# LikeLy-Journey/SegmenTron

Hardware: AMD Instinct MI355X
Metric: images/sec fwd+bwd DeepLabv3+_xception65 @1025x2049 (higher is better)
Workload: dtype bf16; 1 GPU; DeepLabv3+_xception65 train step (fwd + CE loss + bwd + SGD) @1025x2049, batch 2/GPU (BASELINE.json configs[2]); global_batch=2, bn=BN, parallelism=dp1, full_size=True

## Files before the change

segmentron_amd/csrc/dwconv_row.hip:

```cpp
#include "common.h"
#include "dwconv.h"

namespace seg {

constexpr int RW_THREADS = 256, RW_CQ = 8, RW_PL = RW_THREADS / RW_CQ, RW_CH = RW_CQ * 4;

struct DwRowArgs {
  const void* src;
  const void* xc;
  void* out;
  const float* w;
  const float* sc; const float* sh;
  float* partial_a;
  float* partial_bn;
  long ldsrc, ldxc, ldout;
  int N, H, W, C, dil, pro_mode, TW, ntw, ntiles;
};

template <typename T, bool BWD>
__global__ __launch_bounds__(RW_THREADS, BWD ? 2 : 3) void dwconv_row_kernel(const DwRowArgs a) {
  using V = Vec<T>;
  using H4 = HVec<T>;
  constexpr int VN = V::N, VPP = RW_CH / VN;
  constexpr int NACC = BWD ? 9 : 2;
  extern __shared__ __attribute__((aligned(16))) unsigned char rw_smem[];
  T* tile = reinterpret_cast<T*>(rw_smem);
  const int tid = threadIdx.x;
  const int flat = blockIdx.x + gridDim.x * blockIdx.y;
  const int L = xcd_remap(flat, gridDim.x * gridDim.y);
  const int by = L / (int)gridDim.x, bx = L - by * (int)gridDim.x;
  const int cq = tid & (RW_CQ - 1), pl = tid / RW_CQ;
  const int cbase = bx * RW_CH;
  const int c0 = cbase + cq * 4;
  const bool cok = c0 < a.C;
  const int c0s = cok ? c0 : 0;
  const int d = a.dil, TWH = a.TW + 2 * d;
  const T* __restrict__ SRC = reinterpret_cast<const T*>(a.src);
  const T* __restrict__ XC = reinterpret_cast<const T*>(a.xc);
  T* __restrict__ OUT = reinterpret_cast<T*>(a.out);

  const int sv = tid % VPP;
  const int sc0 = cbase + sv * VN;
  const bool sok = sc0 < a.C;
  float ps[VN], pt[VN];
#pragma unroll
  for (int i = 0; i < VN; ++i) { ps[i] = 1.f; pt[i] = 0.f; }
  float sc[4], sh[4];
#pragma unroll
  for (int i = 0; i < 4; ++i) { sc[i] = 1.f; sh[i] = 0.f; }
  if (a.pro_mode & PRO_AFFINE) {
    if (!BWD) {
      load_params<VN>(a.sc, sok ? sc0 : 0, ps);
      load_params<VN>(a.sh, sok ? sc0 : 0, pt);
    } else {
      load_params<4>(a.sc, c0s, sc);
      load_params<4>(a.sh, c0s, sh);
    }
  }
  float wv[9][4];
#pragma unroll
  for (int k = 0; k < 9; ++k) load_params<4>(a.w + (long)k * a.C, c0s, wv[k]);
  float acc[NACC][4], s1[4], s2[4];
#pragma unroll
  for (int k = 0; k < NACC; ++k)
#pragma unroll
    for (int i = 0; i < 4; ++i) acc[k][i] = 0.f;
#pragma unroll
  for (int i = 0; i < 4; ++i) s1[i] = s2[i] = 0.f;

  const int nph = d < a.H ? d : a.H;
  const int nvec_row = TWH * VPP;
  for (int t = by; t < a.ntiles; t += gridDim.y) {
    const int tw = t % a.ntw, tq = t / a.ntw;
    const int ph = tq % nph, n = tq / nph;
    const int w0 = tw * a.TW;
    auto stage_row = [&](int slot, int hh) {
      T* dst = tile + (long)slot * TWH * RW_CH;
      const bool rok = sok && hh >= 0 && hh < a.H;
      for (int idx = tid; idx < nvec_row; idx += RW_THREADS) {
        const int px = idx / VPP;
        const int ww = w0 - d + px;
        const bool ok = rok && ww >= 0 && ww < a.W;
        uint4 v = ldg16(SRC + (ok ? (((long)n * a.H + hh) * a.W + ww) * a.ldsrc + sc0 : 0));
        if (!BWD && a.pro_mode != PRO_NONE) {
          float f[VN];
          V::unpack(v, f);
          apply_prologue_regs<VN>(f, a.pro_mode, ps, pt);
          v = V::pack(f);
        }
        v = mask_u4(v, ok);
        *reinterpret_cast<uint4*>(dst + (long)px * RW_CH + sv * VN) = v;
      }
    };
    __syncthreads();
    stage_row(0, ph - d);
    stage_row(1, ph);
    int k = 0;
    for (int h = ph; h < a.H; h += d, ++k) {
      const long orow = ((long)n * a.H + h) * a.W;
      constexpr int MAXP = (160 + RW_PL - 1) / RW_PL;
      typename H4::raw_t xraw[MAXP];
      if (BWD) {
#pragma unroll
        for (int q = 0; q < MAXP; ++q) {
          const int p = pl + q * RW_PL;
          const bool ok = cok && p < a.TW && w0 + p < a.W;
          xraw[q] = H4::load_raw(XC + (ok ? (orow + w0 + p) * a.ldxc + c0 : 0));
        }
      }
      stage_row((k + 2) % 3, h + d);
      __syncthreads();
      const T* slot_of[3] = {tile + (long)(k % 3) * TWH * RW_CH,
                             tile + (long)((k + 1) % 3) * TWH * RW_CH,
                             tile + (long)((k + 2) % 3) * TWH * RW_CH};
#pragma unroll
      for (int q = 0; q < MAXP; ++q) {
        const int p = pl + q * RW_PL;
        if (!(cok && p < a.TW && w0 + p < a.W)) continue;
        const long poff = (long)(p + d) * RW_CH + cq * 4;
        float o[4] = {0.f, 0.f, 0.f, 0.f};
        if (!BWD) {
#pragma unroll
          for (int kh = 0; kh < 3; ++kh)
#pragma unroll
            for (int kw = 0; kw < 3; ++kw) {
              float f[4];
              H4::load(slot_of[kh] + poff + (long)(kw - 1) * d * RW_CH, f);
#pragma unroll
              for (int i = 0; i < 4; ++i) o[i] = fmaf(f[i], wv[kh * 3 + kw][i], o[i]);
            }
          H4::store(OUT + (orow + w0 + p) * a.ldout + c0, o);
#pragma unroll
          for (int i = 0; i < 4; ++i) {
            acc[0][i] += o[i];
            acc[1][i] = fmaf(o[i], o[i], acc[1][i]);
          }
        } else {
          float xr[4], xa[4];
          H4::unpack_raw(xraw[q], xr);
#pragma unroll
          for (int i = 0; i < 4; ++i) {
            float v = xr[i];
            if (a.pro_mode & PRO_AFFINE) v = fmaf(v, sc[i], sh[i]);
            if (a.pro_mode & PRO_RELU) v = fmaxf(v, 0.f);
            if (a.pro_mode & PRO_CLAMP6) v = fminf(v, 6.f);
            xa[i] = v;
          }
#pragma unroll
          for (int kh = 0; kh < 3; ++kh)
#pragma unroll
            for (int kw = 0; kw < 3; ++kw) {
              float f[4];
              H4::load(slot_of[2 - kh] + poff - (long)(kw - 1) * d * RW_CH, f);
#pragma unroll
              for (int i = 0; i < 4; ++i) {
                o[i] = fmaf(f[i], wv[kh * 3 + kw][i], o[i]);
                acc[kh * 3 + kw][i] = fmaf(f[i], xa[i], acc[kh * 3 + kw][i]);
              }
            }
          if (a.pro_mode & PRO_RELU) {
#pragma unroll
            for (int i = 0; i < 4; ++i) {
              const bool on = xa[i] > 0.f && (!(a.pro_mode & PRO_CLAMP6) || xa[i] < 6.f);
              o[i] = on ? o[i] : 0.f;
            }
          }
          H4::store(OUT + (orow + w0 + p) * a.ldout + c0, o);
#pragma unroll
          for (int i = 0; i < 4; ++i) {
            s1[i] += o[i];
            s2[i] = fmaf(o[i], xr[i], s2[i]);
          }
        }
      }
      __syncthreads();
    }
  }

  constexpr int NR = BWD ? 11 : 2;
  float r[NR][4];
#pragma unroll
  for (int k = 0; k < NACC; ++k)
#pragma unroll
    for (int i = 0; i < 4; ++i) r[k][i] = acc[k][i];
  if (BWD) {
#pragma unroll
    for (int i = 0; i < 4; ++i) { r[NR - 2][i] = s1[i]; r[NR - 1][i] = s2[i]; }
  }
#pragma unroll
  for (int k = 0; k < NR; ++k)
#pragma unroll
    for (int i = 0; i < 4; ++i) {
#pragma unroll
      for (int m = RW_CQ; m < 64; m <<= 1) r[k][i] += __shfl_xor(r[k][i], m, 64);
    }
  __syncthreads();
  float* red = reinterpret_cast<float*>(rw_smem);
  const int wave = tid >> 6;
  if ((tid & 63) < RW_CQ) {
#pragma unroll
    for (int k = 0; k < NR; ++k)
#pragma unroll
      for (int i = 0; i < 4; ++i) red[((wave * RW_CQ + cq) * NR + k) * 4 + i] = r[k][i];
  }
  __syncthreads();
  for (int e = tid; e < RW_CQ * NR * 4; e += RW_THREADS) {
    float tot = 0.f;
#pragma unroll
    for (int wv4 = 0; wv4 < 4; ++wv4) tot += red[wv4 * RW_CQ * NR * 4 + e];
    const int lq = e / (NR * 4), k = (e / 4) % NR, i = e & 3;
    const int c = cbase + lq * 4 + i;
    if (c >= a.C) continue;
    if (!BWD) {
      if (a.partial_a != nullptr) a.partial_a[((long)by * 2 + k) * a.C + c] = tot;
    } else if (k < 9) {
      a.partial_a[((long)by * 9 + k) * a.C + c] = tot;
    } else if (a.partial_bn != nullptr) {
      a.partial_bn[((long)by * 2 + (k - 9)) * a.C + c] = tot;
    }
  }
}

constexpr size_t RW_LDS_MAX = 120 * 1024;

static void row_geom(int dtype, int W, int dil, int& TW, int& ntw) {
  const size_t px_bytes = (size_t)3 * RW_CH * (dtype == DT_BF16 ? 2 : 4);
  ntw = (W + 159) / 160;
  for (;;) {
    TW = (W + ntw - 1) / ntw;
    if ((size_t)(TW + 2 * dil) * px_bytes <= RW_LDS_MAX || TW == 1) break;
    ++ntw;
  }
}

int dw_row_grid_y(int dtype, int C, int N, int H, int W, int dil) {
  int TW, ntw;
  row_geom(dtype, W, dil, TW, ntw);
  const long ntiles = (long)N * (dil < H ? dil : H) * ntw;
  const int gx = (C + RW_CH - 1) / RW_CH;
  long cap = 768 / gx;
  if (cap < 1) cap = 1;
  return (int)(ntiles < cap ? ntiles : cap);
}

template <typename T, bool BWD>
static int launch_row(DwRowArgs a, int dtype, int grid_y, hipStream_t st) {
  row_geom(dtype, a.W, a.dil, a.TW, a.ntw);
  a.ntiles = a.N * (a.dil < a.H ? a.dil : a.H) * a.ntw;
  const size_t tile_b = (size_t)3 * (a.TW + 2 * a.dil) * RW_CH * sizeof(T);
  const size_t red_b = (size_t)4 * RW_CQ * (BWD ? 11 : 2) * 4 * sizeof(float);
  const size_t lds = tile_b > red_b ? tile_b : red_b;
  SEG_REQUIRE(lds <= RW_LDS_MAX, "dwconv3x3 (row): %zu bytes of LDS for dil=%d", lds, a.dil);
  static const int once = (int)hipFuncSetAttribute(
      reinterpret_cast<const void*>(&dwconv_row_kernel<T, BWD>),
      hipFuncAttributeMaxDynamicSharedMemorySize, (int)RW_LDS_MAX);
  if (once != 0) {
    set_error("dwconv3x3 (row): cannot reserve %zu bytes of LDS", RW_LDS_MAX);
    return 2;
  }
  const dim3 grid((a.C + RW_CH - 1) / RW_CH, grid_y);
  hipLaunchKernelGGL((dwconv_row_kernel<T, BWD>), grid, dim3(RW_THREADS), lds, st, a);
  return check_launch(BWD ? "dwconv3x3_bwd_fused (row)" : "dwconv3x3 (row)");
}

int launch_dw_row_fwd(int dtype, const void* x, long ldx, int N, int H, int W, int C,
                      const float* w9c, int dil, int pro_mode, const float* sc, const float* sh,
                      void* y, long ldy, float* stat_partial, int grid_y, hipStream_t st) {
  SEG_REQUIRE(grid_y == dw_row_grid_y(dtype, C, N, H, W, dil), "dwconv3x3 (row): grid_y %d != %d",
              grid_y, dw_row_grid_y(dtype, C, N, H, W, dil));
  DwRowArgs a = {};
  a.src = x; a.out = y; a.w = w9c; a.sc = sc; a.sh = sh; a.partial_a = stat_partial;
  a.ldsrc = ldx; a.ldout = ldy; a.N = N; a.H = H; a.W = W; a.C = C; a.dil = dil;
  a.pro_mode = pro_mode;
  if (dtype == DT_BF16) return launch_row<bf16_t, false>(a, dtype, grid_y, st);
  return launch_row<float, false>(a, dtype, grid_y, st);
}

int launch_dw_row_bwd(int dtype, const void* dy, long lddy, const void* x, long ldx, int N, int H,
                      int W, int C, const float* w9c, int dil, int pro_mode, const float* sc,
                      const float* sh, void* g, long ldg, float* partial_w, float* partial_bn,
                      int grid_y, hipStream_t st) {
  SEG_REQUIRE(grid_y == dw_row_grid_y(dtype, C, N, H, W, dil),
              "dwconv3x3_bwd_fused (row): grid_y %d != %d", grid_y,
              dw_row_grid_y(dtype, C, N, H, W, dil));
  DwRowArgs a = {};
  a.src = dy; a.xc = x; a.out = g; a.w = w9c; a.sc = sc; a.sh = sh;
  a.partial_a = partial_w; a.partial_bn = partial_bn;
  a.ldsrc = lddy; a.ldxc = ldx; a.ldout = ldg; a.N = N; a.H = H; a.W = W; a.C = C; a.dil = dil;
  a.pro_mode = pro_mode;
  if (dtype == DT_BF16) return launch_row<bf16_t, true>(a, dtype, grid_y, st);
  return launch_row<float, true>(a, dtype, grid_y, st);
}

}
```

Baseline: 92.21 images/sec.

## Software-pipeline row dwconv with register-staged loads, 4-slot LDS ring, LDS taps

Reworks the row-tiled depthwise 3x3 kernel so the global loads for the next input row go into registers before the current row's compute, and are written to LDS only afterward. A 4-slot LDS ring is used when it fits, which removes one barrier per row. For bf16 backward, the 9 taps and the BN affine are moved from registers into LDS so three blocks can fit per CU instead of two. Output stores are deferred until after compute and offsets become 32-bit. The cost is more template variants (NV), more code complexity, and extra LDS reads per tap in the backward path.

```diff
diff --git a/segmentron_amd/csrc/dwconv_row.hip b/segmentron_amd/csrc/dwconv_row.hip
--- a/segmentron_amd/csrc/dwconv_row.hip
+++ b/segmentron_amd/csrc/dwconv_row.hip
@@ -1,9 +1,13 @@
+#include <type_traits>
+
 #include "common.h"
 #include "dwconv.h"
 
 namespace seg {
 
 constexpr int RW_THREADS = 256, RW_CQ = 8, RW_PL = RW_THREADS / RW_CQ, RW_CH = RW_CQ * 4;
+constexpr int RW_MAXTW = 160, RW_MAXDIL = 64;
+constexpr int RW_MAXTWH = RW_MAXTW + 2 * RW_MAXDIL;
 
 struct DwRowArgs {
   const void* src;
@@ -14,17 +18,43 @@
   float* partial_a;
   float* partial_bn;
   long ldsrc, ldxc, ldout;
-  int N, H, W, C, dil, pro_mode, TW, ntw, ntiles;
+  int N, H, W, C, dil, pro_mode, TW, ntw, ntiles, nslot;
 };
 
-template <typename T, bool BWD>
-__global__ __launch_bounds__(RW_THREADS, BWD ? 2 : 3) void dwconv_row_kernel(const DwRowArgs a) {
+#ifndef RW_BWD_BF16_BLOCKS
+#define RW_BWD_BF16_BLOCKS 3
+#endif
+#ifndef RW_RING_SLOTS
+#define RW_RING_SLOTS 4
+#endif
+template <typename T, bool BWD, int NV> constexpr int row_blocks_per_cu() {
+  if (sizeof(T) == 4) return (BWD || NV > 6) ? 2 : 3;
+  return BWD ? RW_BWD_BF16_BLOCKS : 3;
+}
+template <typename T, bool BWD> constexpr bool row_taps_in_lds() {
+  return BWD && sizeof(T) == 2 && RW_BWD_BF16_BLOCKS == 3;
+}
+
+__device__ __forceinline__ int opaque(int v) {
+  asm volatile("" : "+v"(v));
+  return v;
+}
+
+__device__ __forceinline__ void arrived(const uint4& v) {
+  asm volatile("" ::"v"(v.x), "v"(v.y), "v"(v.z), "v"(v.w));
+}
+__device__ __forceinline__ void arrived(const uint2& v) { asm volatile("" ::"v"(v.x), "v"(v.y)); }
+
+template <typename T, bool BWD, int NV>
+__global__ __launch_bounds__(RW_THREADS, (row_blocks_per_cu<T, BWD, NV>())) void dwconv_row_kernel(const DwRowArgs a) {
+  constexpr bool WLDS = row_taps_in_lds<T, BWD>();
   using V = Vec<T>;
   using H4 = HVec<T>;
+  using raw_t = typename H4::raw_t;
   constexpr int VN = V::N, VPP = RW_CH / VN;
   constexpr int NACC = BWD ? 9 : 2;
+  constexpr int MAXP = (RW_MAXTW + RW_PL - 1) / RW_PL;
   extern __shared__ __attribute__((aligned(16))) unsigned char rw_smem[];
-  T* tile = reinterpret_cast<T*>(rw_smem);
   const int tid = threadIdx.x;
   const int flat = blockIdx.x + gridDim.x * blockIdx.y;
   const int L = xcd_remap(flat, gridDim.x * gridDim.y);
@@ -34,7 +64,10 @@
   const int c0 = cbase + cq * 4;
   const bool cok = c0 < a.C;
   const int c0s = cok ? c0 : 0;
-  const int d = a.dil, TWH = a.TW + 2 * d;
+  const int d = a.dil, TWH = a.TW + 2 * d, ns = a.nslot;
+  const int slot_elems = TWH * RW_CH;
+  T* tile = reinterpret_cast<T*>(rw_smem);
+  float* wl = reinterpret_cast<float*>(rw_smem + (size_t)ns * slot_elems * sizeof(T));
   const T* __restrict__ SRC = reinterpret_cast<const T*>(a.src);
   const T* __restrict__ XC = reinterpret_cast<const T*>(a.xc);
   T* __restrict__ OUT = reinterpret_cast<T*>(a.out);
@@ -52,14 +85,23 @@
     if (!BWD) {
       load_params<VN>(a.sc, sok ? sc0 : 0, ps);
       load_params<VN>(a.sh, sok ? sc0 : 0, pt);
-    } else {
+    } else if (!WLDS) {
       load_params<4>(a.sc, c0s, sc);
       load_params<4>(a.sh, c0s, sh);
     }
   }
-  float wv[9][4];
-#pragma unroll
-  for (int k = 0; k < 9; ++k) load_params<4>(a.w + (long)k * a.C, c0s, wv[k]);
+  float wv[WLDS ? 1 : 9][4];
+  if constexpr (!WLDS) {
+#pragma unroll
+    for (int k = 0; k < 9; ++k) load_params<4>(a.w + (long)k * a.C, c0s, wv[k]);
+  } else if (tid < 11 * RW_CQ) {
+    const int k = tid / RW_CQ, q = tid % RW_CQ;
+    const int c = cbase + q * 4;
+    float t4[4] = {0.f, 0.f, 0.f, 0.f};
+    if (k < 9) load_params<4>(a.w + (long)k * a.C, c < a.C ? c : 0, t4);
+    else if (a.pro_mode & PRO_AFFINE) load_params<4>(k == 9 ? a.sc : a.sh, c < a.C ? c : 0, t4);
+    *reinterpret_cast<float4*>(wl + k * RW_CH + q * 4) = make_float4(t4[0], t4[1], t4[2], t4[3]);
+  }
   float acc[NACC][4], s1[4], s2[4];
 #pragma unroll
   for (int k = 0; k < NACC; ++k)
@@ -74,62 +116,104 @@
     const int tw = t % a.ntw, tq = t / a.ntw;
     const int ph = tq % nph, n = tq / nph;
     const int w0 = tw * a.TW;
-    auto stage_row = [&](int slot, int hh) {
-      T* dst = tile + (long)slot * TWH * RW_CH;
-      const bool rok = sok && hh >= 0 && hh < a.H;
-      for (int idx = tid; idx < nvec_row; idx += RW_THREADS) {
-        const int px = idx / VPP;
-        const int ww = w0 - d + px;
-        const bool ok = rok && ww >= 0 && ww < a.W;
-        uint4 v = ldg16(SRC + (ok ? (((long)n * a.H + hh) * a.W + ww) * a.ldsrc + sc0 : 0));
-        if (!BWD && a.pro_mode != PRO_NONE) {
-          float f[VN];
-          V::unpack(v, f);
-          apply_prologue_regs<VN>(f, a.pro_mode, ps, pt);
-          v = V::pack(f);
+    auto stage_load = [&](uint4 (&v)[NV], int hh) {
+      const char* rowp = reinterpret_cast<const char*>(SRC + ((long)n * a.H + hh) * a.W * a.ldsrc);
+      const int tv = opaque(tid);
+      const int svc = cbase + (tv % VPP) * VN;
+#pragma unroll
+      for (int j = 0; j < NV; ++j) {
+        const int idx = tv + j * RW_THREADS;
+        const int ww = w0 - d + idx / VPP;
+        const bool ok = svc < a.C && idx < nvec_row && ww >= 0 && ww < a.W;
+        const unsigned off = ok ? (unsigned)(ww * (int)a.ldsrc + svc) * (unsigned)sizeof(T) : 0u;
+        v[j] = ldg16(rowp + off);
+      }
+    };
+    auto stage_write = [&](const uint4 (&v)[NV], bool row_in, int slot) {
+      if (row_in) {
+#pragma unroll
+        for (int j = 0; j < NV; ++j) arrived(v[j]);
+      }
+      const int tv = opaque(tid);
+      T* dst = tile + slot * slot_elems + tv * VN;
+#pragma unroll
+      for (int j = 0; j < NV; ++j) {
+        const int idx = tv + j * RW_THREADS;
+        if (idx < nvec_row) {
+          uint4 o = make_uint4(0u, 0u, 0u, 0u);
+          if (row_in) {
+            const int ww = w0 - d + idx / VPP;
+            o = v[j];
+            if (!BWD && a.pro_mode != PRO_NONE) {
+              float f[VN];
+              V::unpack(o, f);
+              apply_prologue_regs<VN>(f, a.pro_mode, ps, pt);
+              o = V::pack(f);
+            }
+            o = mask_u4(o, cbase + (tv % VPP) * VN < a.C && ww >= 0 && ww < a.W);
+          }
+          *reinterpret_cast<uint4*>(dst + j * (RW_THREADS / VPP) * RW_CH) = o;
         }
-        v = mask_u4(v, ok);
-        *reinterpret_cast<uint4*>(dst + (long)px * RW_CH + sv * VN) = v;
       }
     };
+    auto load_x = [&](raw_t (&xr)[MAXP], int h) {
+      const char* rowp = reinterpret_cast<const char*>(XC + (((long)n * a.H + h) * a.W + w0) * a.ldxc);
+      const int tv = opaque(tid);
+      const int cx = cbase + (tv & (RW_CQ - 1)) * 4;
+#pragma unroll
+      for (int q = 0; q < MAXP; ++q) {
+        const int p = tv / RW_CQ + q * RW_PL;
+        const bool ok = cx < a.C && p < a.TW && w0 + p < a.W;
+        const unsigned off = ok ? (unsigned)(p * (int)a.ldxc + cx) * (unsigned)sizeof(T) : 0u;
+        xr[q] = H4::load_raw(reinterpret_cast<const T*>(rowp + off));
+      }
+    };
+
+    uint4 rv[NV];
+    raw_t xcur[BWD ? MAXP : 1];
+    {
+      uint4 rv2[NV];
+      const bool in2 = ph + d < a.H;
+      stage_load(rv, ph);
+      if (in2) stage_load(rv2, ph + d);
+      if constexpr (BWD) load_x(xcur, ph);
+      stage_write(rv, false, 0);
+      stage_write(rv, true, 1);
+      stage_write(rv2, in2, 2);
+    }
     __syncthreads();
-    stage_row(0, ph - d);
-    stage_row(1, ph);
-    int k = 0;
-    for (int h = ph; h < a.H; h += d, ++k) {
+    int r = 0;
+    auto step = [&](auto in3_c, int h) {
+      constexpr bool IN3 = decltype(in3_c)::value;
+      const int r1 = r + 1 < ns ? r + 1 : r + 1 - ns, r2 = r + 2 < ns ? r + 2 : r + 2 - ns;
+      const int r3 = r + 3 < ns ? r + 3 : r + 3 - ns;
+      const bool more = IN3 || h + d < a.H;
       const long orow = ((long)n * a.H + h) * a.W;
-      constexpr int MAXP = (160 + RW_PL - 1) / RW_PL;
-      typename H4::raw_t xraw[MAXP];
-      if (BWD) {
-#pragma unroll
-        for (int q = 0; q < MAXP; ++q) {
-          const int p = pl + q * RW_PL;
-          const bool ok = cok && p < a.TW && w0 + p < a.W;
-          xraw[q] = H4::load_raw(XC + (ok ? (orow + w0 + p) * a.ldxc + c0 : 0));
-        }
-      }
-      stage_row((k + 2) % 3, h + d);
-      __syncthreads();
-      const T* slot_of[3] = {tile + (long)(k % 3) * TWH * RW_CH,
-                             tile + (long)((k + 1) % 3) * TWH * RW_CH,
-                             tile + (long)((k + 2) % 3) * TWH * RW_CH};
+      if constexpr (IN3) stage_load(rv, h + 2 * d);
+      const T* slot_of[3] = {tile + r * slot_elems, tile + r1 * slot_elems, tile + r2 * slot_elems};
+      raw_t og[MAXP];
+      if constexpr (BWD) {
+#pragma unroll
+        for (int q = 0; q < MAXP; ++q) arrived(xcur[q]);
+      }
 #pragma unroll
       for (int q = 0; q < MAXP; ++q) {
-        const int p = pl + q * RW_PL;
+        const int tv = opaque(tid);
+        const int p = tv / RW_CQ + q * RW_PL;
         if (!(cok && p < a.TW && w0 + p < a.W)) continue;
-        const long poff = (long)(p + d) * RW_CH + cq * 4;
+        const int poff = (p + d) * RW_CH + (tv & (RW_CQ - 1)) * 4;
         float o[4] = {0.f, 0.f, 0.f, 0.f};
-        if (!BWD) {
+        asm volatile("" ::: "memory");
+        if constexpr (!BWD) {
 #pragma unroll
           for (int kh = 0; kh < 3; ++kh)
 #pragma unroll
             for (int kw = 0; kw < 3; ++kw) {
               float f[4];
-              H4::load(slot_of[kh] + poff + (long)(kw - 1) * d * RW_CH, f);
+              H4::load(slot_of[kh] + poff + (kw - 1) * d * RW_CH, f);
 #pragma unroll
               for (int i = 0; i < 4; ++i) o[i] = fmaf(f[i], wv[kh * 3 + kw][i], o[i]);
             }
-          H4::store(OUT + (orow + w0 + p) * a.ldout + c0, o);
 #pragma unroll
           for (int i = 0; i < 4; ++i) {
             acc[0][i] += o[i];
@@ -137,7 +221,15 @@
           }
         } else {
           float xr[4], xa[4];
-          H4::unpack_raw(xraw[q], xr);
+          H4::unpack_raw(xcur[q], xr);
+          if constexpr (WLDS) {
+            if (a.pro_mode & PRO_AFFINE) {
+              const float4 s4 = *reinterpret_cast<const float4*>(wl + 9 * RW_CH + (tv & (RW_CQ - 1)) * 4);
+              const float4 h4 = *reinterpret_cast<const float4*>(wl + 10 * RW_CH + (tv & (RW_CQ - 1)) * 4);
+              sc[0] = s4.x; sc[1] = s4.y; sc[2] = s4.z; sc[3] = s4.w;
+              sh[0] = h4.x; sh[1] = h4.y; sh[2] = h4.z; sh[3] = h4.w;
+            }
+          }
 #pragma unroll
           for (int i = 0; i < 4; ++i) {
             float v = xr[i];
@@ -147,17 +239,27 @@
             xa[i] = v;
           }
 #pragma unroll
-          for (int kh = 0; kh < 3; ++kh)
+          for (int kh = 0; kh < 3; ++kh) {
 #pragma unroll
             for (int kw = 0; kw < 3; ++kw) {
               float f[4];
-              H4::load(slot_of[2 - kh] + poff - (long)(kw - 1) * d * RW_CH, f);
+              H4::load(slot_of[2 - kh] + poff - (kw - 1) * d * RW_CH, f);
+              float wk[4];
+              if constexpr (WLDS) {
+                const float4 w4 = *reinterpret_cast<const float4*>(wl + (kh * 3 + kw) * RW_CH + (tv & (RW_CQ - 1)) * 4);
+                wk[0] = w4.x; wk[1] = w4.y; wk[2] = w4.z; wk[3] = w4.w;
+              } else {
+#pragma unroll
+                for (int i = 0; i < 4; ++i) wk[i] = wv[WLDS ? 0 : kh * 3 + kw][i];
+              }
 #pragma unroll
               for (int i = 0; i < 4; ++i) {
-                o[i] = fmaf(f[i], wv[kh * 3 + kw][i], o[i]);
+                o[i] = fmaf(f[i], wk[i], o[i]);
                 acc[kh * 3 + kw][i] = fmaf(f[i], xa[i], acc[kh * 3 + kw][i]);
               }
             }
+            if constexpr (WLDS) __builtin_amdgcn_sched_barrier(0);
+          }
           if (a.pro_mode & PRO_RELU) {
 #pragma unroll
             for (int i = 0; i < 4; ++i) {
@@ -165,16 +267,35 @@
               o[i] = on ? o[i] : 0.f;
             }
           }
-          H4::store(OUT + (orow + w0 + p) * a.ldout + c0, o);
 #pragma unroll
           for (int i = 0; i < 4; ++i) {
             s1[i] += o[i];
             s2[i] = fmaf(o[i], xr[i], s2[i]);
           }
         }
+        og[q] = H4::pack_raw(o);
+      }
+      if (more) {
+        if (ns == 3) __syncthreads();
+        stage_write(rv, IN3, r3);
+      }
+      char* outp = reinterpret_cast<char*>(OUT + (orow + w0) * a.ldout);
+      const int tvd = opaque(tid);
+#pragma unroll
+      for (int q = 0; q < MAXP; ++q) {
+        const int p = tvd / RW_CQ + q * RW_PL;
+        if (!(cok && p < a.TW && w0 + p < a.W)) continue;
+        *reinterpret_cast<raw_t*>(outp + (unsigned)(p * (int)a.ldout + c0) * (unsigned)sizeof(T)) = og[q];
+      }
+      if constexpr (BWD) {
+        if (more) load_x(xcur, h + d);
       }
       __syncthreads();
-    }
+      r = r1;
+    };
+    int h = ph;
+    for (; h + 2 * d < a.H; h += d) step(std::true_type{}, h);
+    for (; h < a.H; h += d) step(std::false_type{}, h);
   }
 
   constexpr int NR = BWD ? 11 : 2;
@@ -222,6 +343,8 @@
 }
 
 constexpr size_t RW_LDS_MAX = 120 * 1024;
+constexpr size_t RW_LDS_THIRD = 52 * 1024;
+constexpr size_t RW_TAPS_B = (size_t)11 * RW_CH * sizeof(float);
 
 static void row_geom(int dtype, int W, int dil, int& TW, int& ntw) {
   const size_t px_bytes = (size_t)3 * RW_CH * (dtype == DT_BF16 ? 2 : 4);
@@ -243,24 +366,42 @@
   return (int)(ntiles < cap ? ntiles : cap);
 }
 
+template <typename T, bool BWD, int NV>
+static int launch_row_nv(const DwRowArgs& a, size_t lds, const dim3& grid, hipStream_t st) {
+  static const int once = (int)hipFuncSetAttribute(
+      reinterpret_cast<const void*>(&dwconv_row_kernel<T, BWD, NV>),
+      hipFuncAttributeMaxDynamicSharedMemorySize, (int)(RW_LDS_MAX + RW_TAPS_B));
+  if (once != 0) {
+    set_error("dwconv3x3 (row): cannot reserve %zu bytes of LDS", RW_LDS_MAX + RW_TAPS_B);
+    return 2;
+  }
+  hipLaunchKernelGGL((dwconv_row_kernel<T, BWD, NV>), grid, dim3(RW_THREADS), lds, st, a);
+  return check_launch(BWD ? "dwconv3x3_bwd_fused (row)" : "dwconv3x3 (row)");
+}
+
 template <typename T, bool BWD>
 static int launch_row(DwRowArgs a, int dtype, int grid_y, hipStream_t st) {
   row_geom(dtype, a.W, a.dil, a.TW, a.ntw);
   a.ntiles = a.N * (a.dil < a.H ? a.dil : a.H) * a.ntw;
-  const size_t tile_b = (size_t)3 * (a.TW + 2 * a.dil) * RW_CH * sizeof(T);
+  constexpr int VPP = RW_CH / Vec<T>::N;
+  constexpr int NV_MAX = (RW_MAXTWH * VPP + RW_THREADS - 1) / RW_THREADS;
+  constexpr int NV_ASPP = (192 * VPP + RW_THREADS - 1) / RW_THREADS;
+  const int TWH = a.TW + 2 * a.dil;
+  SEG_REQUIRE(a.TW <= RW_MAXTW && a.dil <= RW_MAXDIL, "dwconv3x3 (row): segment of %d pixels, dil=%d",
+              a.TW, a.dil);
+  SEG_REQUIRE((long)a.W * (a.ldsrc > a.ldout ? a.ldsrc : a.ldout) * (long)sizeof(T) < (1L << 31) &&
+                  (long)a.W * a.ldxc * (long)sizeof(T) < (1L << 31),
+              "dwconv3x3 (row): a row of %d pixels spans 2^31 bytes or more", a.W);
+  const size_t slot_b = (size_t)TWH * RW_CH * sizeof(T);
+  const size_t taps_b = row_taps_in_lds<T, BWD>() ? RW_TAPS_B : 0;
+  a.nslot = (RW_RING_SLOTS == 4 && 4 * slot_b + taps_b <= RW_LDS_THIRD) ? 4 : 3;
+  const size_t tile_b = a.nslot * slot_b + taps_b;
   const size_t red_b = (size_t)4 * RW_CQ * (BWD ? 11 : 2) * 4 * sizeof(float);
   const size_t lds = tile_b > red_b ? tile_b : red_b;
-  SEG_REQUIRE(lds <= RW_LDS_MAX, "dwconv3x3 (row): %zu bytes of LDS for dil=%d", lds, a.dil);
-  static const int once = (int)hipFuncSetAttribute(
-      reinterpret_cast<const void*>(&dwconv_row_kernel<T, BWD>),
-      hipFuncAttributeMaxDynamicSharedMemorySize, (int)RW_LDS_MAX);
-  if (once != 0) {
-    set_error("dwconv3x3 (row): cannot reserve %zu bytes of LDS", RW_LDS_MAX);
-    return 2;
-  }
+  SEG_REQUIRE(lds <= RW_LDS_MAX + RW_TAPS_B, "dwconv3x3 (row): %zu bytes of LDS for dil=%d", lds, a.dil);
   const dim3 grid((a.C + RW_CH - 1) / RW_CH, grid_y);
-  hipLaunchKernelGGL((dwconv_row_kernel<T, BWD>), grid, dim3(RW_THREADS), lds, st, a);
-  return check_launch(BWD ? "dwconv3x3_bwd_fused (row)" : "dwconv3x3 (row)");
+  if (TWH * VPP <= NV_ASPP * RW_THREADS) return launch_row_nv<T, BWD, NV_ASPP>(a, lds, grid, st);
+  return launch_row_nv<T, BWD, NV_MAX>(a, lds, grid, st);
 }
 
 int launch_dw_row_fwd(int dtype, const void* x, long ldx, int N, int H, int W, int C,
```

After: 92.61 images/sec (median of 6 runs). Within noise of the previous version (+0.4%).
